# pacificclimate/VIC

Measured on AMD Instinct MI355X. Metric: cell-timesteps/s, higher is better.
Workload: dtype f64

## Files before the change

include/vicgpu.h:

```cpp
#ifndef VICGPU_H_
#define VICGPU_H_

#include <stddef.h>

#ifdef __cplusplus
extern "C" {
#endif

#define VICGPU_ABI_VERSION 3

#define VIC_NLAYER        3
#define VIC_MAX_NODES    50
#define VIC_MAX_BANDS    30
#define VIC_N_PET_TYPES   6
#define VIC_MAX_ZWTVMOIST 11

#define VICGPU_OK               0
#define VICGPU_ERR_ARG         -1
#define VICGPU_ERR_UNSUPPORTED -2
#define VICGPU_ERR_HIP         -3
#define VICGPU_ERR_STATE       -4
#define VICGPU_ERR_NOMEM       -5

#define VIC_SNOW_ALBEDO_USACE   0
// ... 271 lines not shown
  VICGPU_PURE_NFN_DEVICE
};
#define VICGPU_PURE_NIN 10
int   vicgpu_debug_pure(vicgpu_ctx *ctx, int fn, int n, const double *in, double *out);

enum { VICGPU_NODE_NODE1 = 1, VICGPU_NODE_NEWTON = 2, VICGPU_NODE_EXP_TRANS = 4 };
#define VICGPU_NODE_NIN 14
#define VICGPU_NODE_NOUT 2
int   vicgpu_debug_node_root(vicgpu_ctx *ctx, int mode, int n, const double *in, double *out);

enum { VICGPU_BRENT_FULL = 0, VICGPU_BRENT_LEAN = 1 };
#define VICGPU_BRENT_NOUT 9
int   vicgpu_debug_root_brent(vicgpu_ctx *ctx, int mode, int n, const double *bounds, const int *off, const double *fvals,
                              double *xreq, double *out);

int   vicgpu_last_kernel_ms(vicgpu_ctx *ctx, double *ms_per_launch, int *nlaunch);

#ifdef __cplusplus
}
#endif
#endif
```

vic_amd/api.py:

```python
import ctypes
import os

import numpy as np

from . import abi
from .abi import C

_HERE = os.path.dirname(os.path.abspath(__file__))
LIB_PATH = os.path.join(_HERE, "libvicgpu.so")

_dp = ctypes.POINTER(ctypes.c_double)
_ip = ctypes.POINTER(ctypes.c_int)
_up = ctypes.POINTER(ctypes.c_ubyte)

_lib = None


class VicGpuError(RuntimeError):
    pass


def load_library():
    global _lib
    if _lib is not None:
# ... 15 lines not shown
        "vicgpu_push_forcing": (ctypes.c_int, [vp, ctypes.c_int, _dp, _up, _ip]),
        "vicgpu_step": (ctypes.c_int, [vp, ctypes.c_int, ctypes.c_int]),
        "vicgpu_synchronize": (ctypes.c_int, [vp]),
        "vicgpu_get_fluxes": (ctypes.c_int, [vp, _dp]),
        "vicgpu_get_cell_outputs": (ctypes.c_int, [vp, _dp]),
        "vicgpu_get_accum": (ctypes.c_int, [vp, _dp]),
        "vicgpu_reset_accum": (ctypes.c_int, [vp]),
        "vicgpu_get_cell_errors": (ctypes.c_int, [vp, _ip]),
        "vicgpu_set_stream": (ctypes.c_int, [vp, vp]),
        "vicgpu_set_write_fluxes": (ctypes.c_int, [vp, ctypes.c_int]),
        "vicgpu_device_ptr": (vp, [vp, ctypes.c_int]),
        "vicgpu_last_kernel_ms": (ctypes.c_int, [vp, _dp, _ip]),
        "vicgpu_debug_pure": (ctypes.c_int, [vp, ctypes.c_int, ctypes.c_int, _dp, _dp]),
        "vicgpu_debug_node_root": (ctypes.c_int, [vp, ctypes.c_int, ctypes.c_int, _dp, _dp]),
        "vicgpu_debug_root_brent": (ctypes.c_int, [vp, ctypes.c_int, ctypes.c_int, _dp, _ip, _dp, _dp, _dp]),
        "vicgpu_glacier_mass_balance_fit": (ctypes.c_int, [vp, _dp, ctypes.c_int]),
        "vicgpu_prefetch_forcing": (ctypes.c_int, [vp, ctypes.c_int, _dp, _up, _ip]),
        "vicgpu_prefetch_forcing_raw": (ctypes.c_int, [vp, ctypes.c_int, _dp, _ip, ctypes.c_double, ctypes.c_int]),
        "vicgpu_swap_forcing": (ctypes.c_int, [vp]),
        "vicgpu_get_forcing": (ctypes.c_int, [vp, ctypes.c_int, _dp, _up]),
        "vicgpu_host_alloc": (vp, [ctypes.c_size_t]),
        "vicgpu_host_free": (None, [vp]),
        "vicgpu_get_state_records": (ctypes.c_int, [vp, _dp]),
        "vicgpu_set_state_records": (ctypes.c_int, [vp, _dp]),
        "vicgpu_out_nvar": (ctypes.c_int, []),
        "vicgpu_out_var_id": (ctypes.c_int, [ctypes.c_char_p]),
        "vicgpu_out_var_name": (ctypes.c_char_p, [ctypes.c_int]),
        "vicgpu_out_var_kind": (ctypes.c_int, [ctypes.c_int]),
        "vicgpu_out_var_agg": (ctypes.c_int, [ctypes.c_int]),
        "vicgpu_out_var_nelem": (ctypes.c_int, [ctypes.POINTER(abi.Options), ctypes.c_int]),
# ... 39 lines not shown
    _lib = lib
    return lib


GROUP_ENTRIES = [
    "destroy", "last_error", "set_veglib", "set_domain", "set_state", "get_state", "set_fluxes", "get_fluxes", "push_forcing",
    "prefetch_forcing", "prefetch_forcing_raw", "swap_forcing", "step", "synchronize", "put_data_config", "put_data_init",
    "get_outputs", "get_balance", "get_cell_errors", "get_state_records", "set_state_records", "glacier_mass_balance_fit",
]

EXPORTED_SYMBOLS = [
    "vicgpu_abi_version", "vicgpu_create", "vicgpu_destroy", "vicgpu_last_error", "vicgpu_set_veglib", "vicgpu_set_domain",
    "vicgpu_set_state", "vicgpu_get_state", "vicgpu_push_forcing", "vicgpu_step", "vicgpu_synchronize", "vicgpu_get_fluxes",
    "vicgpu_get_cell_outputs", "vicgpu_get_accum", "vicgpu_reset_accum", "vicgpu_get_cell_errors", "vicgpu_set_stream",
    "vicgpu_set_write_fluxes", "vicgpu_device_ptr", "vicgpu_last_kernel_ms", "vicgpu_debug_pure",
    "vicgpu_debug_node_root", "vicgpu_debug_root_brent", "vicgpu_glacier_mass_balance_fit",
    "vicgpu_out_nvar", "vicgpu_out_var_id", "vicgpu_out_var_name", "vicgpu_out_var_kind", "vicgpu_out_var_agg", "vicgpu_out_var_nelem",
    "vicgpu_put_data_config", "vicgpu_put_data_init", "vicgpu_get_outputs", "vicgpu_get_output_data", "vicgpu_get_balance",
    "vicgpu_set_fluxes", "vicgpu_get_state_records", "vicgpu_set_state_records",
    "vicgpu_prefetch_forcing", "vicgpu_prefetch_forcing_raw", "vicgpu_swap_forcing", "vicgpu_get_forcing", "vicgpu_host_alloc",
    "vicgpu_host_free",
] + ["vicgpu_group_" + n for n in GROUP_ENTRIES + ["partition", "create", "shard_bounds", "shard_ctx"]]


def _d(a):
    return a.ctypes.data_as(_dp)


def _i(a):
    return a.ctypes.data_as(_ip)

# ... 200 lines not shown
        assert inp.ndim == 2 and inp.shape[1] == C["VICGPU_NODE_NIN"] and inp.shape[0] > 0
        out = np.zeros((inp.shape[0], C["VICGPU_NODE_NOUT"]))
        self._chk(self.lib.vicgpu_debug_node_root(self.h, int(mode), inp.shape[0], _d(inp), _d(out)))
        return out[:, 0].copy(), out[:, 1] != 0

    def debug_root_brent(self, mode, bounds, fvals, off):
        b = np.ascontiguousarray(bounds, dtype=np.float64)
        f = np.ascontiguousarray(fvals, dtype=np.float64)
        o = np.ascontiguousarray(off, dtype=np.int32)
        assert b.ndim == 2 and b.shape[1] == 2 and b.shape[0] > 0 and o.shape == (b.shape[0] + 1,) and f.shape == (o[-1],)
        x = np.full(max(int(o[-1]), 1), np.nan)
        out = np.zeros((b.shape[0], C["VICGPU_BRENT_NOUT"]))
        self._chk(self.lib.vicgpu_debug_root_brent(self.h, int(mode), b.shape[0], _d(b), _i(o), _d(f) if f.size else None,
                                                   _d(x), _d(out)))
        return x[:o[-1]].copy(), out

    def last_kernel_ms(self):
        ms = ctypes.c_double(0)
        n = ctypes.c_int(0)
        self._chk(self.lib.vicgpu_last_kernel_ms(self.h, ctypes.byref(ms), ctypes.byref(n)))
        return ms.value, n.value


def partition(cell_hru_offset, nshard):
    lib = load_library()
    off = np.ascontiguousarray(cell_hru_offset, dtype=np.int32)
    b = np.zeros(int(nshard) + 1, dtype=np.int32)
    rc = lib.vicgpu_group_partition(len(off) - 1, _i(off), int(nshard), _i(b))
    if rc != 0:
        raise VicGpuError("vicgpu_group_partition failed with code %d" % rc)
# ... 44 lines not shown
```

vic_amd/csrc/vic_profile.hpp:

```cpp
#pragma once
#include "vic_surface.hpp"

namespace vic {

constexpr int NBUCKET = 2 * (VIC_MID_NODES + 2);
static_assert(NBUCKET <= 64, "one lane per work-list segment when the pending total is summed");
constexpr int PEND_STRIPES = 64, PEND_CNT_STRIDE = 32;

struct PArgs {
  const double* __restrict__ pin;
  const double* __restrict__ ts;
  double* __restrict__ pout;
  const int* __restrict__ pslot;
  const int* __restrict__ list;
  const int* __restrict__ count;
  int cap;
  int* next;
  int* count_zero;
  const int* pend_counts;
  const int* pend_stripes;
  int* pend_stripes_zero;
  int* pend_prefix;
  int* pend_out;
  int Nn, NOFLUX, EXP_TRANS, TFALLBACK;
  const int* jl;
};

__host__ __device__ inline int pout_stride(int Nn) { return Nn + 1 + (Nn + 1) / 2; }
__host__ __device__ inline int pout_hru_stride(int Nn) { return 2 * pout_stride(Nn) + 2; }
__host__ __device__ inline int pout_key(int Nn, int slot) { return 2 * pout_stride(Nn) + slot; }

constexpr int LOCKSTEP_GATE = 16;
// ... 177 lines not shown
    } else ok = false;
  }
}

VIC_DEV int profile_pick(const PArgs& a, const int* bcount, int slot) {
  int rem = slot, found = 0;
#pragma unroll 1
  for (int b = NBUCKET - 1; b >= 0; b--) {
    const int cb = bcount[b];
    if (rem < cb) { found = b * a.cap + rem; break; }
    rem -= cb;
  }
  return a.list[found];
}

static_assert(PEND_STRIPES == 64, "one lane per stripe");
VIC_DEV void pend_pack(const PArgs& a, int lane, int keyed_total) {
  a.pend_stripes_zero[lane * PEND_CNT_STRIDE] = 0;
  const int cnt = a.pend_stripes[lane * PEND_CNT_STRIDE];
  int incl = cnt;
#pragma unroll
  for (int off = 1; off < 64; off <<= 1) {
    const int up = __shfl(incl, lane >= off ? lane - off : lane);
    if (lane >= off) incl += up;
  }
  a.pend_prefix[lane + 1] = incl;
  if (lane == 0) a.pend_prefix[0] = 0;
  const int total = __shfl(incl, 63);
  if (lane == 0) *a.pend_out = total > 0 ? total : keyed_total;
}

constexpr int PROFILE_REG_WAVES = 2;
template <int NN, bool NEWTON>
__global__ __launch_bounds__(64) VIC_WAVES_PER_EU(PROFILE_REG_WAVES, PROFILE_REG_WAVES) void vic_profile_solve_reg(const PArgs a) {
  __shared__ int bcount[NBUCKET];
  __shared__ double T0l[NN * 64];
  __shared__ double Kl[3 * (NN - 2) * 64];
  const int lane = threadIdx.x;
#define T0(j) T0l[(j) * 64 + lane]
#define KL(f, j) Kl[((f) * (NN - 2) + (j) - 1) * 64 + lane]
  for (int b = lane; b < NBUCKET; b += 64) bcount[b] = a.count[b];
  if (blockIdx.x == 0) {
    for (int b = lane; b < NBUCKET; b += 64) a.count_zero[b] = 0;
    int v = (lane < NBUCKET) ? a.pend_counts[lane] : 0;
#pragma unroll
    for (int off = 32; off >= 1; off >>= 1) v += __shfl(v, lane ^ off);
    pend_pack(a, lane, v);
  }
  __syncthreads();
  int n = 0;
#pragma unroll
  for (int b = 0; b < NBUCKET; b++) n += bcount[b];
  if ((int)blockIdx.x * 64 >= n) return;

  constexpr int Nn = NN;
  const int jlast = a.NOFLUX ? Nn : Nn - 1;
  const int MAXIT = 1000;
  const double threshold = 1.e-2;
  const bool EXP_TRANS = a.EXP_TRANS != 0;

  bool have = false, sweeping = false, converged = false, ok = true, frozen_on = false;
  int hru = 0, ps = 0, it = 1, jl_lane = 0;
  unsigned fbmask = 0;
  int evcnt = 0;
  double T[NN];
  double kAT0[NN - 1], kB[NN - 1], kC[NN - 1], kD[NN - 1], kEI[NN - 1], kS[NN - 1], kEMM[NN - 1];
#pragma unroll
  for (int k = 0; k < NN; k++) T[k] = 0;
#pragma unroll
  for (int k = 0; k < NN - 1; k++) { kAT0[k] = 0; kB[k] = 0; kC[k] = 0; kD[k] = 0; kEI[k] = 0; kS[k] = 1; kEMM[k] = 0; }
  bool more = true;
  while (true) {
    const unsigned long long idle = __ballot(!have);
    if (more && (__popcll(idle) >= LOCKSTEP_GATE || idle == ~0ull)) {
      PROF_T0(t_gate);
      const int nidle = __popcll(idle), leader = __ffsll((long long)idle) - 1;
      int base = 0;
      if (lane == leader) base = atomicAdd(a.next, nidle);
      base = __builtin_amdgcn_readlane(base, leader);
      if (base + nidle >= n) more = false;
      const int slot = base + __popcll(idle & ((1ull << lane) - 1ull));
      if (!have && slot < n) {
        hru = profile_pick(a, bcount, slot);
        const double* __restrict__ blk = static_cast<const double*>(__builtin_assume_aligned(a.pin + (size_t)hru * Nn * PREC, 16));
        ps = a.pslot[hru];
        jl_lane = a.jl ? a.jl[hru] : jlast;
        frozen_on = blk[PR_AT0] != 0.0;
        const double Ts = a.ts[hru];
#pragma unroll
        for (int k = 0; k < NN; k++) { const double t = (k == 0) ? Ts : blk[k * PREC + PR_T0]; T0(k) = t; T[k] = t; }
#pragma unroll
        for (int k = 1; k < NN - 1; k++) {
          const double* __restrict__ r = blk + k * PREC;
          kAT0[k] = r[PR_AT0]; kB[k] = r[PR_B]; kC[k] = r[PR_C]; kD[k] = r[PR_D]; kEI[k] = r[PR_EI]; kS[k] = r[PR_S]; kEMM[k] = r[PR_EMM];
          KL(0, k) = r[PR_G]; KL(1, k) = r[PR_Y]; KL(2, k) = r[PR_EMOIST];
        }
        have = true; fbmask = 0; evcnt = 0; ok = true; it = 1;
        converged = (jlast <= 1);
        sweeping = !converged;
      }
      PROF_ADD(20, t_gate);
    }
    if (!__any(have)) break;
    PROF_T0(t_sweep);
    {
      double maxdiff = threshold;
      PROF_WAVE(16); PROF_VOTE(17, sweeping);
#pragma unroll
      for (int j = 1; j < NN; j++) {
        if (j < jlast) {
          const double oldT = T[j];
          const double Tdn = (j == Nn - 1) ? oldT : T[(j + 1 < NN) ? j + 1 : j], Tup = T[j - 1];
          const double T0j = T0(j);
          NodeK Kj;
          if (j == NN - 1) Kj.load(a.pin + ((size_t)hru * Nn + j) * PREC);
// ... 55 lines not shown
      }
      a.pout[(size_t)hru * pout_hru_stride(Nn) + pout_key(Nn, ps)] = T0(0);
      have = false;
    }
    PROF_ADD(24, t_fin);
  }
#undef T0
#undef KL
}

constexpr int LS_WAVES = 2;
template <int NN, bool NEWTON>
__global__ __launch_bounds__(64) VIC_WAVES_PER_EU(LS_WAVES, LS_WAVES) void vic_profile_solve_lockstep(const PArgs a) {
  using mask_t = typename NodeBound<NN>::mask_t;
  constexpr bool T0_LDS = NN <= VIC_MID_NODES;
  __shared__ int bcount[NBUCKET];
  __shared__ double Tl[NN * 64];
  __shared__ double T0l[T0_LDS ? NN * 64 : 1];
  const int lane = threadIdx.x;
#define T(j) Tl[(j) * 64 + lane]
#define T0(j) (T0_LDS ? T0l[(T0_LDS ? (j) : 0) * 64 + lane] : ((j) == 0 ? T0s : blk[(j) * PREC + PR_T0]))
  for (int b = lane; b < NBUCKET; b += 64) bcount[b] = a.count[b];
  if (blockIdx.x == 0) {
    for (int b = lane; b < NBUCKET; b += 64) a.count_zero[b] = 0;
    int v = (lane < NBUCKET) ? a.pend_counts[lane] : 0;
#pragma unroll
    for (int off = 32; off >= 1; off >>= 1) v += __shfl(v, lane ^ off);
    pend_pack(a, lane, v);
  }
  __syncthreads();
  int n = 0;
#pragma unroll
  for (int b = 0; b < NBUCKET; b++) n += bcount[b];
  if ((int)blockIdx.x * 64 >= n) return;

  const int Nn = node_count<NN>(a.Nn);
  const int jlast = a.NOFLUX ? Nn : Nn - 1;
  const int MAXIT = 1000;
  const double threshold = 1.e-2;
  const bool EXP_TRANS = a.EXP_TRANS != 0;

#define LS_REC() (a.pout + (size_t)hru * pout_hru_stride(Nn) + ps * pout_stride(Nn))
#define LS_CNT(j) (reinterpret_cast<int*>(LS_REC() + Nn + 1)[j])
  bool have = false, sweeping = false, converged = false, ok = true, frozen_on = false;
  int hru = 0, ps = 0, it = 1, jl_lane = 0;
  mask_t fbmask = 0;
  const double* __restrict__ blk = a.pin;
  double T0s = 0;
  bool more = true;
  while (true) {
    const unsigned long long idle = __ballot(!have);
    if (more && (__popcll(idle) >= LOCKSTEP_GATE || idle == ~0ull)) {
      const int nidle = __popcll(idle), leader = __ffsll((long long)idle) - 1;
      int base = 0;
      if (lane == leader) base = atomicAdd(a.next, nidle);
      base = __builtin_amdgcn_readlane(base, leader);
      if (base + nidle >= n) more = false;
      const int slot = base + __popcll(idle & ((1ull << lane) - 1ull));
      if (!have && slot < n) {
        hru = profile_pick(a, bcount, slot);
        blk = a.pin + (size_t)hru * Nn * PREC;
        ps = a.pslot[hru];
        jl_lane = a.jl ? a.jl[hru] : jlast;
        frozen_on = blk[PR_AT0] != 0.0;
        const double Ts = a.ts[hru];
#pragma unroll
        for (int k = 0; k < NN; k++)
          if (k < Nn) {
            const double t = (k == 0) ? Ts : blk[k * PREC + PR_T0];
            if constexpr (T0_LDS) T0l[k * 64 + lane] = t;
            T(k) = t; LS_CNT(k) = 0;
          }
        T0s = Ts;
        have = true; fbmask = 0; ok = true; it = 1;
        converged = (jlast <= 1);
        sweeping = !converged;
      }
    }
    if (!__any(have)) break;
    {
      double maxdiff = threshold;
      PROF_WAVE(16); PROF_VOTE(17, sweeping);
#pragma unroll 1
      for (int j = 1; j < NN; j++) {
        if (j < jlast) {
          double oldT = 0, Tdn = 0, Tup = 0, T0j = 0;
          NodeK K;
          K.AT0 = 0; K.B = 0; K.C = 0; K.D = 0; K.EI = 0; K.S = 1; K.G = 0; K.Y = 0; K.EM = 0; K.EMM = 0;
          if (sweeping) {
            oldT = T(j);
            Tdn = (j == Nn - 1) ? oldT : T((j + 1 < NN) ? j + 1 : j); Tup = T(j - 1);
            T0j = T0(j);
// ... 62 lines not shown
```

vic_amd/csrc/vic_types.hpp:

```cpp
#pragma once
#include <hip/hip_runtime.h>
#include <math.h>
#include <limits.h>
#include "vicgpu.h"

#define VIC_DEV __device__ __forceinline__
#define VIC_DEVN __device__ __forceinline__
#ifdef VIC_HOSTEMU
#define VIC_WAVES_PER_EU(lo, hi)
#else
#define VIC_WAVES_PER_EU(lo, hi) __attribute__((amdgpu_waves_per_eu(lo, hi)))
#endif

namespace vic {

constexpr int VIC_MID_NODES = 24;
static_assert(VIC_MID_NODES < VIC_MAX_NODES && VIC_MAX_NODES <= 63, "node bounds");
template <bool B, class T, class F> struct vic_cond { using type = T; };
template <class T, class F> struct vic_cond<false, T, F> { using type = F; };
__host__ __device__ constexpr int node_bound(int Nnode) { return Nnode == 10 ? 10 : (Nnode <= VIC_MID_NODES ? VIC_MID_NODES : VIC_MAX_NODES); }
__host__ __device__ constexpr int record_ok_bit(int bound) { return bound > 32 ? 63 : 32; }
template <int NN> struct NodeBound {
  static constexpr bool generic = (NN == VIC_MID_NODES || NN == VIC_MAX_NODES);
  using mask_t = typename vic_cond<(NN > 32), unsigned long long, unsigned>::type;
// ... 45 lines not shown
constexpr double MIN_SWQ_EB_THRES = 0.0010;
constexpr double TRACESNOW = 0.03;
constexpr int NPET = 6;
constexpr int NPET_NON_NAT = 4;
constexpr int PET_VEGNOCR = 5;

enum { SNOW_FREE = 0, CANOPY = 1, SNOW_COVERED = 2, GLACIER_SURF = 3, NCASE = 4 };

#ifdef VIC_PROF
__device__ unsigned long long vic_prof_cyc[32];
__device__ unsigned long long vic_prof_cnt[32];
VIC_DEV bool prof_leader() { return (int)__lane_id() == __ffsll((long long)__ballot(1)) - 1; }
#define PROF_T0(name) const long long name = (long long)__builtin_readcyclecounter()
#define PROF_ADD(id, name) do { const long long _d = (long long)__builtin_readcyclecounter() - (name); \
    if (prof_leader()) atomicAdd(&vic_prof_cyc[id], (unsigned long long)_d); } while (0)
#define PROF_LANE(id) atomicAdd(&vic_prof_cnt[id], 1ull)
#define PROF_WAVE(id) do { if (prof_leader()) atomicAdd(&vic_prof_cnt[id], 1ull); } while (0)
#define PROF_VOTE(id, pred) do { const unsigned long long m_ = __ballot(pred); if (prof_leader()) atomicAdd(&vic_prof_cnt[id], (unsigned long long)__popcll(m_)); } while (0)
#else
#define PROF_T0(name) do { } while (0)
#define PROF_ADD(id, name) do { } while (0)
#define PROF_LANE(id) do { } while (0)
#define PROF_WAVE(id) do { } while (0)
#define PROF_VOTE(id, pred) do { } while (0)
#endif

VIC_DEV bool is_error(double x) { return x <= -998.0; }

struct Opt {
  int Nnode, Nband, dt, snow_step, NF, NR;
  int FULL_ENERGY, FROZEN_SOIL, QUICK_FLUX, NOFLUX, EXP_TRANS, GRND_FLUX_TYPE, TFALLBACK, AERO_RESIST_CANSNOW,
      SNOW_ALBEDO, SNOW_DENSITY, TEMP_TH_TYPE, GLACIER_ID, GLACIER_DYNAMICS, frozen_compat, nveg_types, CORRPREC, IMPLICIT, QUICK_SOLVE, BLOWING;
  double wind_h;
};

struct VegLib {
// ... 79 lines not shown
```

vic_amd/csrc/vicgpu_api.hip:

```cpp
#include <hip/hip_runtime.h>
#include <stdio.h>
#include <stdlib.h>
#include <string.h>
#include <algorithm>
#include <atomic>
#include <chrono>
#include <memory>
#include <string>
#include <thread>
#include <vector>
#include "vicgpu.h"
#include <cstddef>
#include <type_traits>
#include "vic_glacier.hpp"
#include "vic_profile.hpp"
#include "vic_putdata.hpp"
#include "vic_host.hpp"

using namespace vic;

#define HIPIGN(call) do { hipError_t ign_ = (call); (void)ign_; } while (0)
#define HIPCHK(ctx, call)                                                                              \
  do {                                                                                                 \
    hipError_t e_ = (call);                                                                            \
// ... 1289 lines not shown
    DevBuf<unsigned char> d_s;
    PinnedBuf<char> h_stage;
    std::vector<int> dmy;
    int nsteps = 0;
    Event uploaded;
    Event released;
    bool upload_pending = false, was_current = false;
  } slot[2];
  int cur = -1, staged = -1;
  Stream stream, copy_stream;
  std::vector<Event> ev;
  int ev_used = 0;
  int write_fluxes = 1;
  int steps_done = 0;
  int profile_waves = 0;
  int eval_list_pct = 75;
  bool node_newton = false;
  int ev_steps = 0;
  int out_step_ratio = 1;
};

static void free_domain(vicgpu_ctx* c) {
  c->dom = Domain();
  c->chunk_steps = 0;
  c->dmy.clear();
  c->cur = c->staged = -1;
  c->d_forcing = nullptr; c->d_snowflag = nullptr;
}

template <int NN>
// ... 7 lines not shown
}

template <int NN>
static hipError_t launch_fd_stage(const KArgs& ka, bool multi, hipStream_t st) {
  const dim3 grid(ka.map.nblocks(ka.gcount)), block(64);
  if (ka.phase == 0) {
    if (multi) hipLaunchKernelGGL((vic_fd_stage<NN, true, true>), grid, block, 0, st, ka);
    else hipLaunchKernelGGL((vic_fd_stage<NN, true, false>), grid, block, 0, st, ka);
  } else {
    if (multi) hipLaunchKernelGGL((vic_fd_stage<NN, false, true>), grid, block, 0, st, ka);
    else hipLaunchKernelGGL((vic_fd_stage<NN, false, false>), grid, block, 0, st, ka);
  }
  return hipGetLastError();
}

template <int NN>
static hipError_t launch_profile(const PArgs& pa, int nmax, int resident_waves, bool newton, hipStream_t st) {
  int nblk = (nmax + 63) / 64;
  if (nblk > resident_waves) nblk = resident_waves;
  if (nblk < 1) nblk = 1;
  const dim3 g(nblk), b(64);
  if constexpr (NN == 10) {
    if (newton) hipLaunchKernelGGL((vic_profile_solve_reg<NN, true>), g, b, 0, st, pa);
    else hipLaunchKernelGGL((vic_profile_solve_reg<NN, false>), g, b, 0, st, pa);
  } else {
    if (newton) hipLaunchKernelGGL((vic_profile_solve_lockstep<NN, true>), g, b, 0, st, pa);
    else hipLaunchKernelGGL((vic_profile_solve_lockstep<NN, false>), g, b, 0, st, pa);
  }
  return hipGetLastError();
}

template <int NN>
static int profile_resident_waves(int device, bool newton) {
  int per_cu = 0, ncu = 0;
  hipError_t e;
// ... 30 lines not shown
#define NODE_DISPATCH(Nnode, F, ...)                                                                                          \
  (node_bound(Nnode) == 10 ? F<10>(__VA_ARGS__)                                                                           \
                           : node_bound(Nnode) == VIC_MID_NODES ? F<VIC_MID_NODES>(__VA_ARGS__) : F<VIC_MAX_NODES>(__VA_ARGS__))

static int fd_step(vicgpu_ctx* c, FdChunk* ch, KArgs ka) {
  const int Nn = c->o.Nnode;
  hipStream_t st = ch->stream;
  if (c->dom.any_glacier) HIPCHK(ch, NODE_DISPATCH(Nn, launch_hru, ka, st, false, true));
  HIPCHK(ch, hipMemsetAsync(ch->d_count, 0, sizeof(int) * CNT_TOTAL, st));
  int cur = 0;
  ka.phase = 0; ka.list = ch->d_list[cur]; ka.count = cnt_list(ch->d_count, cur); ka.list_cap = ch->list_cap;
  HIPCHK(ch, NODE_DISPATCH(Nn, launch_fd_stage, ka, c->o.NF > 1, st));
  PArgs pa;
  pa.pin = c->dom.d_pin; pa.ts = c->dom.d_ts; pa.pout = c->dom.d_pout; pa.pslot = c->dom.d_pslot; pa.Nn = Nn; pa.NOFLUX = c->o.NOFLUX; pa.EXP_TRANS = c->o.EXP_TRANS;
  pa.TFALLBACK = c->o.TFALLBACK; pa.next = ch->d_count + CNT_CURSOR; pa.cap = ch->list_cap; pa.jl = c->dom.d_jl;
  EArgs ea;
  ea.o = c->o; ea.ncell = c->dom.ncell; ea.nhru = c->dom.nhru; ea.Nn = Nn; ea.glist = ch->d_glist; ea.gcount = ch->gcount; ea.map = ch->map;
  ea.cell_params = c->dom.d_cp; ea.hpi = c->dom.d_hpi; ea.ctx = c->dom.d_ctx;
  ea.ctx_words = NODE_DISPATCH(Nn, ctx_words);
  ea.pout = c->dom.d_pout; ea.pslot = c->dom.d_pslot; ea.ts = c->dom.d_ts; ea.hstate = c->dom.d_hstate; ea.profile_next = ch->d_count + CNT_CURSOR;
  const int list_thr = (int)((long long)ch->gcount * c->eval_list_pct / 100);
  ea.pend_cap = ch->pend_cap;
  ea.list_cap = ch->list_cap; ea.hkey = c->dom.d_hkey; ea.implicit = c->o.IMPLICIT; ea.jl = c->dom.d_jl;
  ea.veglib = c->d_veglib; ea.forcing = ka.forcing; ea.month = ka.dmy.month;
  const bool trace_rounds = getenv("VICGPU_TRACE_ROUNDS") != nullptr;
  const int FREE_ROUNDS = 6;
  const int nsub = c->o.NF;
  for (int p = 1; p <= nsub; p++) {
    int nmax = ch->gcount;
    int npend = -1;
// ... 5 lines not shown
      pa.pend_stripes_zero = cnt_stripes(ch->d_count, cur ^ 1); pa.pend_prefix = ch->d_count + CNT_PREFIX; pa.pend_out = ch->d_count + CNT_NPEND;
      if (c->o.IMPLICIT) {
        HIPCHK(ch, hipMemsetAsync(ch->d_fb_count, 0, sizeof(int) * (NBUCKET + 1), st));
        IArgs ia;
        ia.ncell = c->dom.ncell; ia.nhru = c->dom.nhru; ia.Nband = c->o.Nband; ia.pimp = c->dom.d_pimp; ia.hpi = c->dom.d_hpi; ia.cell_params = c->dom.d_cp;
        ia.hkey = c->dom.d_hkey; ia.fb_list = ch->d_fb_list; ia.fb_count = ch->d_fb_count; ia.lastexp = c->dom.d_lastexp; ia.cursor = ch->d_fb_count + NBUCKET;
        {
          int nblk = (nmax + 63) / 64;
          if (nblk > 4096) nblk = 4096;
          if (nblk < 1) nblk = 1;
          hipLaunchKernelGGL(vic_profile_solve_implicit, dim3(nblk), dim3(64), 0, st, pa, ia);
        }
        HIPCHK(ch, hipGetLastError());
        pa.list = ch->d_fb_list; pa.count = ch->d_fb_count;
      }
      HIPCHK(ch, NODE_DISPATCH(Nn, launch_profile, pa, nmax, c->profile_waves, c->node_newton, st));
      ea.list_next = ch->d_list[cur ^ 1]; ea.count_next = cnt_list(ch->d_count, cur ^ 1);
      ea.pend_list_next = ch->d_plist[cur ^ 1]; ea.pend_count_next = cnt_stripes(ch->d_count, cur ^ 1);
      ea.pend_list_cur = ch->d_plist[cur]; ea.pend_prefix = ch->d_count + CNT_PREFIX; ea.npend_cur = ch->d_count + CNT_NPEND;
      ea.list_thr = round > 0 ? list_thr : -1;
      const bool sparse = npend >= 0 && npend <= ea.list_thr;
      hipLaunchKernelGGL(vic_surf_eval, dim3(sparse ? ((npend + 63) / 64 > 0 ? (npend + 63) / 64 : 1) : ea.map.nblocks(ch->gcount)), dim3(64), 0, st, ea);
      HIPCHK(ch, hipGetLastError());
      cur ^= 1;
      ch->rounds++;
      if (trace_rounds) {
        int n = 0, np = 0;
        if (fd_read_count(ch, cur, &n, &np) != VICGPU_OK) return VICGPU_ERR_HIP;
        fprintf(stderr, "vicgpu rounds: chunk %d sub-step %d round %d leaves %d solves + %d evaluation-only of %d\n", (int)(ch - &c->dom.chunks[0]), p, round, n, np - n, ch->gcount);
      }
      if (round + 2 >= FREE_ROUNDS) {
// ... 249 lines not shown
    c->node_newton = c->opt.NODE_SOLVER == VIC_NODE_SOLVER_NEWTON;
    if (const char* ev = getenv("VICGPU_NODE_SOLVER")) c->node_newton = (strcmp(ev, "newton") == 0);
    c->profile_waves = NODE_DISPATCH(Nn, profile_resident_waves, c->device, c->node_newton);
    if (const char* ev = getenv("VICGPU_EVAL_LIST_PCT")) {
      const int pct = atoi(ev);
      if (pct >= 0 && pct <= 100) c->eval_list_pct = pct;
    }
    int nchunk = (ncell >= 20000) ? 2 : 1;
    if (const char* ev = getenv("VICGPU_CHUNKS")) nchunk = atoi(ev);
    if (nchunk < 1) nchunk = 1;
    if (nchunk > 16) nchunk = 16;
    if (nchunk > ncell) nchunk = ncell;
    int waves_pct = nchunk > 1 ? 50 : 100;
    if (const char* ev = getenv("VICGPU_PROFILE_WAVES_PCT")) {
      const int pct = atoi(ev);
      if (pct >= 5 && pct <= 100) waves_pct = pct;
    }
    c->profile_waves = c->profile_waves * waves_pct / 100 > 0 ? c->profile_waves * waves_pct / 100 : 1;
    c->dom.chunks.resize(nchunk);
    for (int k = 0; k < nchunk; k++) {
      FdChunk& ch = c->dom.chunks[k];
      ch.c0 = (int)((long long)ncell * k / nchunk);
      ch.ccount = (int)((long long)ncell * (k + 1) / nchunk) - ch.c0;
      std::vector<int> gl(cell_hru_list + cell_hru_offset[ch.c0], cell_hru_list + cell_hru_offset[ch.c0 + ch.ccount]);
      std::sort(gl.begin(), gl.end());
      ch.gcount = (int)gl.size();
      ch.map = LaunchMap();
      if (ch.ccount > 0 && ch.gcount % ch.ccount == 0 && !getenv("VICGPU_NO_XCD_MAP")) {
        const int nslot = ch.gcount / ch.ccount;
        bool regular = true;
        for (int sl = 0; sl < nslot && regular; sl++)
// ... 435 lines not shown
  NRArgs d;
  d.n = n; d.EXP_TRANS = (mode & VICGPU_NODE_EXP_TRANS) != 0; d.in = d_in; d.out = d_out;
  const dim3 grid((n + 63) / 64), block(64);
  switch (mode & (VICGPU_NODE_NODE1 | VICGPU_NODE_NEWTON)) {
    case 0: hipLaunchKernelGGL((vic_debug_node_root<false, false>), grid, block, 0, c->stream, d); break;
    case VICGPU_NODE_NODE1: hipLaunchKernelGGL((vic_debug_node_root<true, false>), grid, block, 0, c->stream, d); break;
    case VICGPU_NODE_NEWTON: hipLaunchKernelGGL((vic_debug_node_root<false, true>), grid, block, 0, c->stream, d); break;
    default: hipLaunchKernelGGL((vic_debug_node_root<true, true>), grid, block, 0, c->stream, d); break;
  }
  HIPCHK(c, hipGetLastError());
  HIPCHK(c, hipStreamSynchronize(c->stream));
  HIPCHK(c, copy_on(c->stream, out, d_out, sizeof(double) * (size_t)n * VICGPU_NODE_NOUT, hipMemcpyDeviceToHost));
  return VICGPU_OK;
}

int vicgpu_set_stream(vicgpu_ctx* c, void* hip_stream) {
  if (!c) return VICGPU_ERR_ARG;
  HIPCHK(c, hipSetDevice(c->device));
  HIPCHK(c, hipStreamSynchronize(c->stream));
  if (hip_stream) c->stream.borrow((hipStream_t)hip_stream);
  else if (c->stream.borrowed()) HIPCHK(c, c->stream.create());
  return VICGPU_OK;
}

int vicgpu_set_write_fluxes(vicgpu_ctx* c, int on) {
  if (!c) return VICGPU_ERR_ARG;
  c->write_fluxes = on ? 1 : 0;
  return VICGPU_OK;
}

// ... 198 lines not shown
```

Measured before the change: 4.133 million.

## Prefetch profile-solve work in 64-entry blocks via double-buffered LDS take queue

Replaces the per-gate atomicAdd plus bucket binary search in the profile solve kernels with a WorkTake helper. Each wave reserves blocks of 64 list entries ahead of time, resolves the HRU ids into a double-buffered LDS queue, and hands them out to idle lanes. Near the end of the list (the tail) it falls back to fine-grained atomic takes to keep load balanced. The aim is to hide the latency of the global atomic and list loads behind compute, at the cost of extra LDS state, synchronisation and code complexity. Also adds a debug kernel, API and env knobs for testing take correctness.

```diff
diff --git a/include/vicgpu.h b/include/vicgpu.h
--- a/include/vicgpu.h
+++ b/include/vicgpu.h
@@ -309,6 +309,9 @@
 int   vicgpu_debug_root_brent(vicgpu_ctx *ctx, int mode, int n, const double *bounds, const int *off, const double *fvals,
                               double *xreq, double *out);
 
+#define VICGPU_PROFILE_NSEG 52
+int   vicgpu_debug_profile_take(vicgpu_ctx *ctx, const int *counts, int cap, int nwaves, int block, int tail_slots, int *hits);
+
 int   vicgpu_last_kernel_ms(vicgpu_ctx *ctx, double *ms_per_launch, int *nlaunch);
 
 #ifdef __cplusplus
diff --git a/vic_amd/api.py b/vic_amd/api.py
--- a/vic_amd/api.py
+++ b/vic_amd/api.py
@@ -53,6 +53,7 @@
         "vicgpu_debug_pure": (ctypes.c_int, [vp, ctypes.c_int, ctypes.c_int, _dp, _dp]),
         "vicgpu_debug_node_root": (ctypes.c_int, [vp, ctypes.c_int, ctypes.c_int, _dp, _dp]),
         "vicgpu_debug_root_brent": (ctypes.c_int, [vp, ctypes.c_int, ctypes.c_int, _dp, _ip, _dp, _dp, _dp]),
+        "vicgpu_debug_profile_take": (ctypes.c_int, [vp, _ip, ctypes.c_int, ctypes.c_int, ctypes.c_int, ctypes.c_int, _ip]),
         "vicgpu_glacier_mass_balance_fit": (ctypes.c_int, [vp, _dp, ctypes.c_int]),
         "vicgpu_prefetch_forcing": (ctypes.c_int, [vp, ctypes.c_int, _dp, _up, _ip]),
         "vicgpu_prefetch_forcing_raw": (ctypes.c_int, [vp, ctypes.c_int, _dp, _ip, ctypes.c_double, ctypes.c_int]),
@@ -122,7 +123,7 @@
     "vicgpu_set_state", "vicgpu_get_state", "vicgpu_push_forcing", "vicgpu_step", "vicgpu_synchronize", "vicgpu_get_fluxes",
     "vicgpu_get_cell_outputs", "vicgpu_get_accum", "vicgpu_reset_accum", "vicgpu_get_cell_errors", "vicgpu_set_stream",
     "vicgpu_set_write_fluxes", "vicgpu_device_ptr", "vicgpu_last_kernel_ms", "vicgpu_debug_pure",
-    "vicgpu_debug_node_root", "vicgpu_debug_root_brent", "vicgpu_glacier_mass_balance_fit",
+    "vicgpu_debug_node_root", "vicgpu_debug_root_brent", "vicgpu_debug_profile_take", "vicgpu_glacier_mass_balance_fit",
     "vicgpu_out_nvar", "vicgpu_out_var_id", "vicgpu_out_var_name", "vicgpu_out_var_kind", "vicgpu_out_var_agg", "vicgpu_out_var_nelem",
     "vicgpu_put_data_config", "vicgpu_put_data_init", "vicgpu_get_outputs", "vicgpu_get_output_data", "vicgpu_get_balance",
     "vicgpu_set_fluxes", "vicgpu_get_state_records", "vicgpu_set_state_records",
@@ -353,6 +354,13 @@
         self._chk(self.lib.vicgpu_debug_root_brent(self.h, int(mode), b.shape[0], _d(b), _i(o), _d(f) if f.size else None,
                                                    _d(x), _d(out)))
         return x[:o[-1]].copy(), out
+
+    def debug_profile_take(self, counts, cap, nwaves, block, tail_slots):
+        cnt = np.ascontiguousarray(counts, dtype=np.int32)
+        assert cnt.shape == (C["VICGPU_PROFILE_NSEG"],)
+        hits = np.full((C["VICGPU_PROFILE_NSEG"], int(cap)), -1, dtype=np.int32)
+        self._chk(self.lib.vicgpu_debug_profile_take(self.h, _i(cnt), int(cap), int(nwaves), int(block), int(tail_slots), _i(hits)))
+        return hits
 
     def last_kernel_ms(self):
         ms = ctypes.c_double(0)
diff --git a/vic_amd/csrc/vic_profile.hpp b/vic_amd/csrc/vic_profile.hpp
--- a/vic_amd/csrc/vic_profile.hpp
+++ b/vic_amd/csrc/vic_profile.hpp
@@ -16,6 +16,8 @@
   const int* __restrict__ count;
   int cap;
   int* next;
+  int take_block;
+  int take_tail;
   int* count_zero;
   const int* pend_counts;
   const int* pend_stripes;
@@ -223,6 +225,155 @@
   return a.list[found];
 }
 
+constexpr int TAKE_BLOCK = 64;
+struct WorkTake {
+  enum { ST_RB, ST_POS, ST_CRB, ST_COB, ST_LASTBASE, ST_LCNT, ST_FLAGS, ST_N, ST_CAP, ST_BLOCK, ST_TAIL, ST_WORDS };
+  enum { F_EXHAUSTED = 1, F_A = 2, F_L = 4 };
+  static constexpr int LDS_INTS = 64 + 2 * TAKE_BLOCK + ST_WORDS;
+  int* pre;
+  const int* list;
+  int* next;
+  bool more_;
+  int rbase, rword;
+  int cap, n, block, tail;
+  int rb, pos, c_rb, c_ob;
+  int lastbase, lcnt;
+  bool exhausted, A, L, fresh;
+
+  VIC_DEV int* ids() const { return pre + 64; }
+  VIC_DEV int* st() const { return pre + 64 + 2 * TAKE_BLOCK; }
+  VIC_DEV int init(const PArgs& a, int* lds, int lane) {
+    static_assert(NBUCKET <= 64, "one lane per segment");
+    pre = lds;
+    list = a.list; next = a.next;
+    const int c = (lane < NBUCKET) ? a.count[NBUCKET - 1 - lane] : 0;
+    int incl = c;
+#pragma unroll
+    for (int off = 1; off < 64; off <<= 1) {
+      const int up = __shfl(incl, lane >= off ? lane - off : lane);
+      if (lane >= off) incl += up;
+    }
+    pre[lane] = incl - c;
+    const int total = __shfl(incl, 63);
+    if (lane < ST_WORDS) st()[lane] = (lane == ST_N) ? total : (lane == ST_CAP) ? a.cap : (lane == ST_BLOCK) ? a.take_block : (lane == ST_TAIL) ? a.take_tail : 0;
+    more_ = total > 0;
+    rbase = 0; rword = 0;
+    __syncthreads();
+    return total;
+  }
+  VIC_DEV int word(int k) const { return __builtin_amdgcn_readfirstlane(st()[k]); }
+  VIC_DEV void load() {
+    rb = word(ST_RB); pos = word(ST_POS); c_rb = word(ST_CRB); c_ob = word(ST_COB); lastbase = word(ST_LASTBASE); lcnt = word(ST_LCNT);
+    const int f = word(ST_FLAGS);
+    exhausted = (f & F_EXHAUSTED) != 0; A = (f & F_A) != 0; L = (f & F_L) != 0;
+    n = word(ST_N); cap = word(ST_CAP); block = word(ST_BLOCK); tail = word(ST_TAIL);
+    fresh = false;
+  }
+  VIC_DEV void save(int lane) {
+    if (lane == 0) {
+      int* w = st();
+      w[ST_RB] = rb; w[ST_POS] = pos; w[ST_CRB] = c_rb; w[ST_COB] = c_ob; w[ST_LASTBASE] = lastbase; w[ST_LCNT] = lcnt;
+      w[ST_FLAGS] = (exhausted ? F_EXHAUSTED : 0) | (A ? F_A : 0) | (L ? F_L : 0);
+    }
+    more_ = !exhausted || A || L || c_rb + c_ob > 0;
+    __syncthreads();
+  }
+  VIC_DEV int pick(int slot) const {
+    int p = 0;
+#pragma unroll
+    for (int s = 32; s >= 1; s >>= 1)
+      if (pre[p + s] <= slot) p += s;
+    return (NBUCKET - 1 - p) * cap + (slot - pre[p]);
+  }
+  VIC_DEV bool more() const { return more_; }
+  VIC_DEV bool block_mode() const { return block > 0 && n - lastbase > tail; }
+  VIC_DEV bool can_reserve() const { return !A && !exhausted && block_mode() && c_rb + c_ob + (L ? lcnt : 0) <= TAKE_BLOCK; }
+  VIC_DEV void reserve(int lane) {
+    if (lane == 0) rbase = atomicAdd(next, TAKE_BLOCK);
+    A = true; fresh = true;
+  }
+  VIC_DEV void resolve(int lane) {
+    const int base = __builtin_amdgcn_readfirstlane(rbase);
+    A = false; lastbase = base;
+    if (base + TAKE_BLOCK >= n) exhausted = true;
+    lcnt = base < n ? (n - base < TAKE_BLOCK ? n - base : TAKE_BLOCK) : 0;
+    if (lcnt > 0) {
+      if (lane < lcnt) rword = list[pick(base + lane)];
+      L = true;
+    }
+  }
+  VIC_DEV bool land(int lane) {
+    if (c_rb > 0 && c_ob > 0) return false;
+    const int wb = (c_rb > 0) ? (rb ^ 1) : rb;
+    if (lane < lcnt) ids()[wb * TAKE_BLOCK + lane] = rword;
+    __syncthreads();
+    if (c_rb > 0) c_ob = lcnt;
+    else { c_rb = lcnt; pos = 0; }
+    L = false;
+    return true;
+  }
+  VIC_DEV bool take(unsigned long long idle, int lane, int& hru) {
+    const int need = __popcll(idle), rank = __popcll(idle & ((1ull << lane) - 1ull));
+    const bool want = ((idle >> lane) & 1ull) != 0;
+    load();
+    if (L) land(lane);
+    while (c_rb + c_ob < need) {
+      bool moved = false;
+      if (A && !L) { resolve(lane); moved = true; }
+      if (L && land(lane)) moved = true;
+      if (can_reserve()) { reserve(lane); moved = true; }
+      if (!moved) break;
+    }
+    const int avail = c_rb + c_ob, k = avail < need ? avail : need;
+    bool got = false;
+    if (want && rank < k) {
+      hru = (rank < c_rb) ? ids()[rb * TAKE_BLOCK + pos + rank] : ids()[(rb ^ 1) * TAKE_BLOCK + rank - c_rb];
+      got = true;
+    }
+    if (k < c_rb) { pos += k; c_rb -= k; }
+    else { const int k2 = k - c_rb; rb ^= 1; pos = k2; c_rb = c_ob - k2; c_ob = 0; }
+    const int rest = need - k;
+    if (rest > 0 && !exhausted && !block_mode()) {
+      const bool first = want && rank == k;
+      int base = 0;
+      if (first) base = atomicAdd(next, rest);
+      base = __builtin_amdgcn_readlane(base, __ffsll((long long)__ballot(first)) - 1);
+      lastbase = base;
+      if (base + rest >= n) exhausted = true;
+      const int slot = base + rank - k;
+      if (want && rank >= k && slot < n) { hru = list[pick(slot)]; got = true; }
+    }
+    return got;
+  }
+  VIC_DEV void ahead(int lane) {
+    if (A && !L && !fresh) resolve(lane);
+    if (can_reserve()) reserve(lane);
+    save(lane);
+  }
+};
+
+struct TKArgs {
+  PArgs p;
+  int* hits;
+  int nent;
+};
+__global__ __launch_bounds__(64) void vic_debug_profile_take(const TKArgs t) {
+  __shared__ int take_lds[WorkTake::LDS_INTS];
+  const int lane = threadIdx.x;
+  WorkTake wt;
+  const int n = wt.init(t.p, take_lds, lane);
+  if ((int)blockIdx.x * 64 >= n) return;
+  for (unsigned gate = 0; wt.more() && gate < (unsigned)n + 2u; gate++) {
+    unsigned h = ((unsigned)blockIdx.x * 2654435761u) ^ (gate * 40503u + 0x9E3779B9u) ^ ((unsigned)lane * 2246822519u);
+    h ^= h >> 15; h *= 2246822519u; h ^= h >> 13;
+    unsigned long long idle = __ballot((h & 3u) == 0u);
+    for (int l = 0; __popcll(idle) < LOCKSTEP_GATE; l++) idle |= 1ull << l;
+    if ((gate & 7u) == 0u) idle = ~0ull;
+    int id = -1;
+    if (wt.take(idle, lane, id)) atomicAdd(&t.hits[(id >= 0 && id < t.nent) ? id : t.nent], 1);
+    wt.ahead(lane);
+  }
+}
 static_assert(PEND_STRIPES == 64, "one lane per stripe");
 VIC_DEV void pend_pack(const PArgs& a, int lane, int keyed_total) {
   a.pend_stripes_zero[lane * PEND_CNT_STRIDE] = 0;
@@ -242,13 +393,12 @@
 constexpr int PROFILE_REG_WAVES = 2;
 template <int NN, bool NEWTON>
 __global__ __launch_bounds__(64) VIC_WAVES_PER_EU(PROFILE_REG_WAVES, PROFILE_REG_WAVES) void vic_profile_solve_reg(const PArgs a) {
-  __shared__ int bcount[NBUCKET];
+  __shared__ int take_lds[WorkTake::LDS_INTS];
   __shared__ double T0l[NN * 64];
   __shared__ double Kl[3 * (NN - 2) * 64];
   const int lane = threadIdx.x;
 #define T0(j) T0l[(j) * 64 + lane]
 #define KL(f, j) Kl[((f) * (NN - 2) + (j) - 1) * 64 + lane]
-  for (int b = lane; b < NBUCKET; b += 64) bcount[b] = a.count[b];
   if (blockIdx.x == 0) {
     for (int b = lane; b < NBUCKET; b += 64) a.count_zero[b] = 0;
     int v = (lane < NBUCKET) ? a.pend_counts[lane] : 0;
@@ -256,10 +406,8 @@
     for (int off = 32; off >= 1; off >>= 1) v += __shfl(v, lane ^ off);
     pend_pack(a, lane, v);
   }
-  __syncthreads();
-  int n = 0;
-#pragma unroll
-  for (int b = 0; b < NBUCKET; b++) n += bcount[b];
+  WorkTake wt;
+  const int n = wt.init(a, take_lds, lane);
   if ((int)blockIdx.x * 64 >= n) return;
 
   constexpr int Nn = NN;
@@ -278,19 +426,15 @@
   for (int k = 0; k < NN; k++) T[k] = 0;
 #pragma unroll
   for (int k = 0; k < NN - 1; k++) { kAT0[k] = 0; kB[k] = 0; kC[k] = 0; kD[k] = 0; kEI[k] = 0; kS[k] = 1; kEMM[k] = 0; }
-  bool more = true;
   while (true) {
     const unsigned long long idle = __ballot(!have);
-    if (more && (__popcll(idle) >= LOCKSTEP_GATE || idle == ~0ull)) {
+    if (wt.more() && (__popcll(idle) >= LOCKSTEP_GATE || idle == ~0ull)) {
       PROF_T0(t_gate);
-      const int nidle = __popcll(idle), leader = __ffsll((long long)idle) - 1;
-      int base = 0;
-      if (lane == leader) base = atomicAdd(a.next, nidle);
-      base = __builtin_amdgcn_readlane(base, leader);
-      if (base + nidle >= n) more = false;
-      const int slot = base + __popcll(idle & ((1ull << lane) - 1ull));
-      if (!have && slot < n) {
-        hru = profile_pick(a, bcount, slot);
+      const bool take = wt.take(idle, lane, hru);
+      PROF_WAVE(28); PROF_VOTE(29, !have); PROF_VOTE(30, take);
+      PROF_PIN(hru); PROF_ADD(26, t_gate);
+      PROF_T0(t_load);
+      if (take) {
         const double* __restrict__ blk = static_cast<const double*>(__builtin_assume_aligned(a.pin + (size_t)hru * Nn * PREC, 16));
         ps = a.pslot[hru];
         jl_lane = a.jl ? a.jl[hru] : jlast;
@@ -308,6 +452,8 @@
         converged = (jlast <= 1);
         sweeping = !converged;
       }
+      PROF_PIN(kEMM[NN - 2]); PROF_PIN(ps); PROF_ADD(27, t_load);
+      wt.ahead(lane);
       PROF_ADD(20, t_gate);
     }
     if (!__any(have)) break;
@@ -393,13 +539,12 @@
 __global__ __launch_bounds__(64) VIC_WAVES_PER_EU(LS_WAVES, LS_WAVES) void vic_profile_solve_lockstep(const PArgs a) {
   using mask_t = typename NodeBound<NN>::mask_t;
   constexpr bool T0_LDS = NN <= VIC_MID_NODES;
-  __shared__ int bcount[NBUCKET];
+  __shared__ int take_lds[WorkTake::LDS_INTS];
   __shared__ double Tl[NN * 64];
   __shared__ double T0l[T0_LDS ? NN * 64 : 1];
   const int lane = threadIdx.x;
 #define T(j) Tl[(j) * 64 + lane]
 #define T0(j) (T0_LDS ? T0l[(T0_LDS ? (j) : 0) * 64 + lane] : ((j) == 0 ? T0s : blk[(j) * PREC + PR_T0]))
-  for (int b = lane; b < NBUCKET; b += 64) bcount[b] = a.count[b];
   if (blockIdx.x == 0) {
     for (int b = lane; b < NBUCKET; b += 64) a.count_zero[b] = 0;
     int v = (lane < NBUCKET) ? a.pend_counts[lane] : 0;
@@ -407,10 +552,8 @@
     for (int off = 32; off >= 1; off >>= 1) v += __shfl(v, lane ^ off);
     pend_pack(a, lane, v);
   }
-  __syncthreads();
-  int n = 0;
-#pragma unroll
-  for (int b = 0; b < NBUCKET; b++) n += bcount[b];
+  WorkTake wt;
+  const int n = wt.init(a, take_lds, lane);
   if ((int)blockIdx.x * 64 >= n) return;
 
   const int Nn = node_count<NN>(a.Nn);
@@ -426,18 +569,10 @@
   mask_t fbmask = 0;
   const double* __restrict__ blk = a.pin;
   double T0s = 0;
-  bool more = true;
   while (true) {
     const unsigned long long idle = __ballot(!have);
-    if (more && (__popcll(idle) >= LOCKSTEP_GATE || idle == ~0ull)) {
-      const int nidle = __popcll(idle), leader = __ffsll((long long)idle) - 1;
-      int base = 0;
-      if (lane == leader) base = atomicAdd(a.next, nidle);
-      base = __builtin_amdgcn_readlane(base, leader);
-      if (base + nidle >= n) more = false;
-      const int slot = base + __popcll(idle & ((1ull << lane) - 1ull));
-      if (!have && slot < n) {
-        hru = profile_pick(a, bcount, slot);
+    if (wt.more() && (__popcll(idle) >= LOCKSTEP_GATE || idle == ~0ull)) {
+      if (wt.take(idle, lane, hru)) {
         blk = a.pin + (size_t)hru * Nn * PREC;
         ps = a.pslot[hru];
         jl_lane = a.jl ? a.jl[hru] : jlast;
@@ -455,6 +590,7 @@
         converged = (jlast <= 1);
         sweeping = !converged;
       }
+      wt.ahead(lane);
     }
     if (!__any(have)) break;
     {
diff --git a/vic_amd/csrc/vic_types.hpp b/vic_amd/csrc/vic_types.hpp
--- a/vic_amd/csrc/vic_types.hpp
+++ b/vic_amd/csrc/vic_types.hpp
@@ -83,12 +83,14 @@
 #define PROF_T0(name) const long long name = (long long)__builtin_readcyclecounter()
 #define PROF_ADD(id, name) do { const long long _d = (long long)__builtin_readcyclecounter() - (name); \
     if (prof_leader()) atomicAdd(&vic_prof_cyc[id], (unsigned long long)_d); } while (0)
+#define PROF_PIN(x) asm volatile("" ::"v"(x))
 #define PROF_LANE(id) atomicAdd(&vic_prof_cnt[id], 1ull)
 #define PROF_WAVE(id) do { if (prof_leader()) atomicAdd(&vic_prof_cnt[id], 1ull); } while (0)
 #define PROF_VOTE(id, pred) do { const unsigned long long m_ = __ballot(pred); if (prof_leader()) atomicAdd(&vic_prof_cnt[id], (unsigned long long)__popcll(m_)); } while (0)
 #else
 #define PROF_T0(name) do { } while (0)
 #define PROF_ADD(id, name) do { } while (0)
+#define PROF_PIN(x) do { } while (0)
 #define PROF_LANE(id) do { } while (0)
 #define PROF_WAVE(id) do { } while (0)
 #define PROF_VOTE(id, pred) do { } while (0)
diff --git a/vic_amd/csrc/vicgpu_api.hip b/vic_amd/csrc/vicgpu_api.hip
--- a/vic_amd/csrc/vicgpu_api.hip
+++ b/vic_amd/csrc/vicgpu_api.hip
@@ -1,4 +1,5 @@
 #include <hip/hip_runtime.h>
+#include <limits.h>
 #include <stdio.h>
 #include <stdlib.h>
 #include <string.h>
@@ -1327,6 +1328,8 @@
   int write_fluxes = 1;
   int steps_done = 0;
   int profile_waves = 0;
+  int profile_take = TAKE_BLOCK;
+  int profile_take_tail = 4;
   int eval_list_pct = 75;
   bool node_newton = false;
   int ev_steps = 0;
@@ -1364,11 +1367,17 @@
   return hipGetLastError();
 }
 
+static int profile_take_tail_slots(int tail_blocks, int nwaves) {
+  const long long t = (long long)tail_blocks * TAKE_BLOCK * nwaves;
+  return t > INT_MAX ? INT_MAX : (int)t;
+}
+
 template <int NN>
-static hipError_t launch_profile(const PArgs& pa, int nmax, int resident_waves, bool newton, hipStream_t st) {
+static hipError_t launch_profile(PArgs pa, int nmax, int resident_waves, int tail_blocks, bool newton, hipStream_t st) {
   int nblk = (nmax + 63) / 64;
   if (nblk > resident_waves) nblk = resident_waves;
   if (nblk < 1) nblk = 1;
+  pa.take_tail = profile_take_tail_slots(tail_blocks, nblk);
   const dim3 g(nblk), b(64);
   if constexpr (NN == 10) {
     if (newton) hipLaunchKernelGGL((vic_profile_solve_reg<NN, true>), g, b, 0, st, pa);
@@ -1429,6 +1438,7 @@
   PArgs pa;
   pa.pin = c->dom.d_pin; pa.ts = c->dom.d_ts; pa.pout = c->dom.d_pout; pa.pslot = c->dom.d_pslot; pa.Nn = Nn; pa.NOFLUX = c->o.NOFLUX; pa.EXP_TRANS = c->o.EXP_TRANS;
   pa.TFALLBACK = c->o.TFALLBACK; pa.next = ch->d_count + CNT_CURSOR; pa.cap = ch->list_cap; pa.jl = c->dom.d_jl;
+  pa.take_block = c->profile_take; pa.take_tail = 0;
   EArgs ea;
   ea.o = c->o; ea.ncell = c->dom.ncell; ea.nhru = c->dom.nhru; ea.Nn = Nn; ea.glist = ch->d_glist; ea.gcount = ch->gcount; ea.map = ch->map;
   ea.cell_params = c->dom.d_cp; ea.hpi = c->dom.d_hpi; ea.ctx = c->dom.d_ctx;
@@ -1464,7 +1474,7 @@
         HIPCHK(ch, hipGetLastError());
         pa.list = ch->d_fb_list; pa.count = ch->d_fb_count;
       }
-      HIPCHK(ch, NODE_DISPATCH(Nn, launch_profile, pa, nmax, c->profile_waves, c->node_newton, st));
+      HIPCHK(ch, NODE_DISPATCH(Nn, launch_profile, pa, nmax, c->profile_waves, c->profile_take_tail, c->node_newton, st));
       ea.list_next = ch->d_list[cur ^ 1]; ea.count_next = cnt_list(ch->d_count, cur ^ 1);
       ea.pend_list_next = ch->d_plist[cur ^ 1]; ea.pend_count_next = cnt_stripes(ch->d_count, cur ^ 1);
       ea.pend_list_cur = ch->d_plist[cur]; ea.pend_prefix = ch->d_count + CNT_PREFIX; ea.npend_cur = ch->d_count + CNT_NPEND;
@@ -1744,7 +1754,15 @@
     int waves_pct = nchunk > 1 ? 50 : 100;
     if (const char* ev = getenv("VICGPU_PROFILE_WAVES_PCT")) {
       const int pct = atoi(ev);
-      if (pct >= 5 && pct <= 100) waves_pct = pct;
+      if (pct >= 1 && pct <= 100) waves_pct = pct;
+    }
+    if (const char* ev = getenv("VICGPU_PROFILE_TAKE")) {
+      const int blk = atoi(ev);
+      if (blk == 0 || blk == TAKE_BLOCK) c->profile_take = blk;
+    }
+    if (const char* ev = getenv("VICGPU_PROFILE_TAKE_TAIL")) {
+      const int t = atoi(ev);
+      if (t >= 0) c->profile_take_tail = t;
     }
     c->profile_waves = c->profile_waves * waves_pct / 100 > 0 ? c->profile_waves * waves_pct / 100 : 1;
     c->dom.chunks.resize(nchunk);
@@ -2210,6 +2228,39 @@
   return VICGPU_OK;
 }
 
+static_assert(VICGPU_PROFILE_NSEG == NBUCKET, "vicgpu.h: segments of the keyed work list");
+int vicgpu_debug_profile_take(vicgpu_ctx* c, const int* counts, int cap, int nwaves, int block, int tail_slots, int* hits) {
+  if (!c || !counts || !hits || cap <= 0 || cap > INT_MAX / VICGPU_PROFILE_NSEG || nwaves <= 0 || nwaves > 4096 ||
+      (block != 0 && block != TAKE_BLOCK) || tail_slots < 0)
+    return VICGPU_ERR_ARG;
+  for (int b = 0; b < NBUCKET; b++)
+    if (counts[b] < 0 || counts[b] > cap) return VICGPU_ERR_ARG;
+  HIPCHK(c, hipSetDevice(c->device));
+  const int nent = NBUCKET * cap;
+  std::vector<int> own(nent);
+  for (int i = 0; i < nent; i++) own[i] = i;
+  DevBuf<int> d_list, d_count, d_hits;
+  HIPCHK(c, d_list.alloc(nent));
+  HIPCHK(c, d_count.alloc(NBUCKET + 1));
+  HIPCHK(c, d_hits.alloc((size_t)nent + 1));
+  HIPCHK(c, copy_on(c->stream, d_list, own.data(), sizeof(int) * (size_t)nent, hipMemcpyHostToDevice));
+  HIPCHK(c, fill_on(c->stream, d_count, 0, sizeof(int) * (NBUCKET + 1)));
+  HIPCHK(c, copy_on(c->stream, d_count, counts, sizeof(int) * NBUCKET, hipMemcpyHostToDevice));
+  HIPCHK(c, fill_on(c->stream, d_hits, 0, sizeof(int) * ((size_t)nent + 1)));
+  TKArgs t;
+  memset(&t, 0, sizeof(t));
+  t.p.list = d_list; t.p.count = d_count; t.p.cap = cap; t.p.next = (int*)d_count + NBUCKET; t.p.take_block = block; t.p.take_tail = tail_slots;
+  t.hits = d_hits; t.nent = nent;
+  hipLaunchKernelGGL(vic_debug_profile_take, dim3(nwaves), dim3(64), 0, c->stream, t);
+  HIPCHK(c, hipGetLastError());
+  HIPCHK(c, hipStreamSynchronize(c->stream));
+  std::vector<int> h((size_t)nent + 1);
+  HIPCHK(c, copy_on(c->stream, h.data(), d_hits, sizeof(int) * ((size_t)nent + 1), hipMemcpyDeviceToHost));
+  if (h[nent] != 0) { c->err = "vicgpu_debug_profile_take: a list word outside the list was handed out"; return VICGPU_ERR_HIP; }
+  memcpy(hits, h.data(), sizeof(int) * (size_t)nent);
+  return VICGPU_OK;
+}
+
 int vicgpu_set_stream(vicgpu_ctx* c, void* hip_stream) {
   if (!c) return VICGPU_ERR_ARG;
   HIPCHK(c, hipSetDevice(c->device));
```

Result: slower. 3.989 million (-3.5%).
